# xingyizhou/CenterTrack

Hardware: AMD Instinct MI355X
Metric: frames/sec (DLA-34 + DCNv2 CenterTrack hot path: H2D of the frame + forward + decode + D2H + track association) (higher is better)
Workload: dtype f32; 1 GPU; mot17_512: mot heads, DLA-34, 512x512, 1 stream(s)/GPU, K=100, flip_test=False, seeded random-init weights; one step = 64 consecutive frames of every stream, each frame uploaded from pinned host memory inside the step (frame t+1 on a copy stream while frame t runs); global_batch=1, parallelism=streams sharded dp1, all-gather of packed detections, hip_graph=True

## Files before the change

centertrack_amd/_lib.py:

```python
import ctypes
import os

_PKG = os.path.dirname(os.path.abspath(__file__))
LIB_PATH = os.environ.get('CENTERTRACK_LIB') or os.path.join(_PKG, 'libcentertrack_hip.so')

c_float_p = ctypes.c_void_p
NUM_HEADS = 11
(HEAD_REG, HEAD_WH, HEAD_TRACKING, HEAD_LTRB, HEAD_LTRB_AMODAL, HEAD_DEP, HEAD_ROT, HEAD_DIM,
 HEAD_AMODEL_OFFSET, HEAD_NUSCENES_ATT, HEAD_VELOCITY) = range(NUM_HEADS)
HEAD_INDEX = {'reg': HEAD_REG, 'wh': HEAD_WH, 'tracking': HEAD_TRACKING, 'ltrb': HEAD_LTRB,
              'ltrb_amodal': HEAD_LTRB_AMODAL, 'dep': HEAD_DEP, 'rot': HEAD_ROT, 'dim': HEAD_DIM,
              'amodel_offset': HEAD_AMODEL_OFFSET, 'nuscenes_att': HEAD_NUSCENES_ATT,
              'velocity': HEAD_VELOCITY}
HEAD_CH = {'reg': 2, 'wh': 2, 'tracking': 2, 'ltrb': 4, 'ltrb_amodal': 4, 'dep': 1, 'rot': 8, 'dim': 3,
           'amodel_offset': 2, 'nuscenes_att': 8, 'velocity': 3}

CT_RELU = 1
CT_OUT_NCHW = 2
CT_DCN_MAIN, CT_DCN_FINISH, CT_DCN_OFFSETS = 1, 2, 4
CT_OK, CT_ERR_ARG, CT_ERR_LAUNCH, CT_ERR_WORKSPACE = 0, 1, 2, 3


class ConvDesc(ctypes.Structure):
    _fields_ = [('x', ctypes.c_void_p), ('N', ctypes.c_int), ('H', ctypes.c_int), ('W', ctypes.c_int),
# ... 142 lines not shown
                ('frame', ctypes.c_void_p), ('next_frame', ctypes.c_void_p),
                ('trans_input', ctypes.c_void_p), ('trans_inv', ctypes.c_void_p)]


CT_FRAME_DEVICE, CT_FRAME_HOST, CT_FRAME_IN_PLACE, CT_FRAME_UPLOADED = range(4)


ABI_VERSION = 103

EXPORTS = ['ct_last_error', 'ct_version', 'ct_set_tuning', 'ct_packed_weight_elems', 'ct_pack_conv_weight',
           'ct_packed_winograd_elems', 'ct_pack_winograd_weight', 'ct_conv2d',
           'ct_conv2d_workspace_bytes', 'ct_heads_fused', 'ct_dcn_v2', 'ct_dcn_v2_workspace_bytes', 'ct_dcn_v2_offsets_bytes', 'ct_dcn_v2_group', 'ct_dcn_v2_group_workspace_bytes', 'ct_dcn_v2_group_plan',
           'ct_dcn_v2_backward', 'ct_dcn_v2_backward_workspace_bytes', 'ct_packed_dcn_weight_t_elems', 'ct_pack_dcn_weight_t', 'ct_stem_forward',
           'ct_maxpool2x2', 'ct_upsample_add', 'ct_nchw_to_nhwc', 'ct_nhwc_to_nchw',
           'ct_decode_row_floats', 'ct_decode_workspace_bytes', 'ct_decode', 'ct_decode_pose_workspace_bytes',
           'ct_decode_pose', 'ct_render_pre_hm',
           'ct_tracker_create', 'ct_tracker_destroy', 'ct_tracker_reset', 'ct_tracker_num_tracks',
           'ct_tracker_id_count', 'ct_tracker_get_tracks', 'ct_tracker_step', 'ct_tracker_prehm_params', 'ct_linear_assignment', 'ct_tracker_set_mode', 'ct_tracker_init_tracks',
           'ct_tracker_step_public', 'ct_tracker_step_dets', 'ct_transform_points',
           'ct_preprocess_image', 'ct_preprocess_lut', 'ct_preprocess_device', 'ct_graph_begin', 'ct_graph_end', 'ct_graph_launch', 'ct_graph_destroy',
           'ct_memcpy_async', 'ct_memset_async', 'ct_stream_synchronize', 'ct_flip_merge', 'ct_flip_images',
           'ct_frame_loop_create', 'ct_frame_loop_destroy', 'ct_frame_loop_submit', 'ct_frame_loop_wait', 'ct_frame_loop_finish',
           'ct_frame_loop_finish_submit', 'ct_frame_loop_upload', 'ct_frame_loop_pending_slot', 'ct_frame_loop_in_flight',
           'ct_frame_loop_forget_upload', 'ct_frame_loop_prestage', 'ct_stem_forward_parts', 'ct_signal_host']

_lib = None


class CTError(RuntimeError):
    pass


def load():
    global _lib
    if _lib is not None:
        return _lib
    if not os.path.exists(LIB_PATH):
        raise CTError('%s not found: build it with `python -c "import __graft_entry__ as g; g.build()"` '
                      '(hipcc --offload-arch=gfx950); there is no CPU fallback' % LIB_PATH)
    import torch
    lib = ctypes.CDLL(LIB_PATH)
    i, p, sz = ctypes.c_int, ctypes.c_void_p, ctypes.c_size_t
    lib.ct_last_error.restype = ctypes.c_char_p
    lib.ct_version.restype = i
    if lib.ct_version() != ABI_VERSION:
        raise CTError('%s is ABI version %d, this binding was written against %d: rebuild it (python -m '
                      'centertrack_amd.build)' % (LIB_PATH, lib.ct_version(), ABI_VERSION))
# ... 5 lines not shown
    lib.ct_packed_winograd_elems.argtypes = [i, i]
    lib.ct_pack_winograd_weight.argtypes = [p, p, i, i, p]
    lib.ct_conv2d.argtypes = [ctypes.POINTER(ConvDesc), p]
    lib.ct_conv2d_workspace_bytes.restype = sz
    lib.ct_conv2d_workspace_bytes.argtypes = [ctypes.POINTER(ConvDesc)]
    lib.ct_heads_fused.argtypes = [ctypes.POINTER(HeadsDesc), p]
    lib.ct_dcn_v2.argtypes = [ctypes.POINTER(DcnDesc), p]
    lib.ct_dcn_v2_workspace_bytes.restype = sz
    lib.ct_dcn_v2_workspace_bytes.argtypes = [ctypes.POINTER(DcnDesc)]
    lib.ct_dcn_v2_offsets_bytes.restype = sz
    lib.ct_dcn_v2_offsets_bytes.argtypes = [ctypes.POINTER(DcnDesc)]
    lib.ct_dcn_v2_group.argtypes = [ctypes.POINTER(DcnDesc), i, i, p]
    lib.ct_dcn_v2_group_workspace_bytes.restype = sz
    lib.ct_dcn_v2_group_workspace_bytes.argtypes = [ctypes.POINTER(DcnDesc)]
    lib.ct_dcn_v2_group_plan.argtypes = [ctypes.POINTER(DcnDesc), ctypes.POINTER(ctypes.c_size_t), ctypes.POINTER(ctypes.c_int)]
    lib.ct_dcn_v2_backward.argtypes = [ctypes.POINTER(DcnBwdDesc), p]
    lib.ct_dcn_v2_backward_workspace_bytes.restype = sz
    lib.ct_dcn_v2_backward_workspace_bytes.argtypes = [ctypes.POINTER(DcnBwdDesc)]
    lib.ct_packed_dcn_weight_t_elems.restype = sz
    lib.ct_packed_dcn_weight_t_elems.argtypes = [i, i]
    lib.ct_pack_dcn_weight_t.argtypes = [p, p, i, i, p]
    lib.ct_stem_forward.argtypes = [p, p, p, i, i, i, p, p, p, p, p, p, i, p]
    lib.ct_stem_forward_parts.argtypes = [p, p, p, p, i, i, i, i, p, p, p, p, p, p, i, p]
    lib.ct_maxpool2x2.argtypes = [p, i, i, i, i, i, p, i, p]
    lib.ct_upsample_add.argtypes = [p, i, i, i, i, i, p, i, p, i, p, i, p]
    lib.ct_nchw_to_nhwc.argtypes = [p, i, i, i, i, p, i, p]
    lib.ct_nhwc_to_nchw.argtypes = [p, i, i, i, i, i, p, p]
    lib.ct_decode_row_floats.argtypes = [ctypes.POINTER(DecodeDesc)]
    lib.ct_decode_workspace_bytes.restype = sz
    lib.ct_decode_workspace_bytes.argtypes = [ctypes.POINTER(DecodeDesc)]
    lib.ct_decode.argtypes = [ctypes.POINTER(DecodeDesc), p]
    lib.ct_decode_pose_workspace_bytes.restype = sz
    lib.ct_decode_pose_workspace_bytes.argtypes = [ctypes.POINTER(PoseDesc)]
    lib.ct_decode_pose.argtypes = [ctypes.POINTER(PoseDesc), p]
    lib.ct_render_pre_hm.argtypes = [p, p, i, i, i, i, p, i, p]
    lib.ct_tracker_create.restype = p
    lib.ct_tracker_create.argtypes = [ctypes.c_float, i]
    lib.ct_tracker_destroy.restype = None
    lib.ct_tracker_destroy.argtypes = [p]
    lib.ct_tracker_reset.restype = None
    lib.ct_tracker_reset.argtypes = [p]
    lib.ct_tracker_num_tracks.argtypes = [p]
    lib.ct_tracker_id_count.argtypes = [p]
    lib.ct_tracker_get_tracks.argtypes = [p, p, i]
    lib.ct_tracker_step.argtypes = [p, p, i, i, ctypes.POINTER(RowLayout), ctypes.c_float, p, p, i]
    lib.ct_tracker_prehm_params.argtypes = [p, ctypes.c_float, p, i, i, p, i]
# ... 74 lines not shown
```

centertrack_amd/csrc/stem.hip:

```cpp
#include "ct_common.h"

namespace {

constexpr int ST_TW = 32;
constexpr int ST_PW = 40;
template <int TH> struct StCfg {
    static constexpr int PH = TH + 6;
    static constexpr int PS = PH * ST_PW;
    static constexpr int NPV = (3 * PH * 38 + 255) / 256;
    static constexpr int HALVES = TH / 8;
};
__host__ __device__ constexpr int st_k4(int s) { return s == 2 ? 52 : 148; }
__host__ __device__ constexpr int st_koff(int s) { return s * 148; }
constexpr int ST_KTOT = 348;
constexpr int ST_WLP = 16;

CT_DEFINE_STAMPS(stem)

struct StemArgs {
    const float *in[3];
    const float *w[3];
    const float *scale;
    const float *shift;
    const float *add;
    float *y;
    int N, H, W, ldy, ldadd, tilesX, tilesY;
};

constexpr int ST_NWV = 10;

template <int TH>
__attribute__((amdgpu_waves_per_eu(TH == 16 ? 2 : 1)))
__global__ __launch_bounds__(256) void stem_kernel(StemArgs a)
{
    using SC = StCfg<TH>;
    constexpr int ST_TH = TH, ST_PH = SC::PH, ST_PS = SC::PS, ST_NPV = SC::NPV, MT = 4, HV = SC::HALVES;
    __shared__ __attribute__((aligned(16))) float planes[7 * ST_PS];
    __shared__ __attribute__((aligned(16))) float wl[ST_KTOT * ST_WLP];
    __shared__ int tab[ST_KTOT];
    CT_STAMP_RT(0);
    CT_STAMP(1);
    CT_STAMP_HW(8);

    const int tid = threadIdx.x;
    const int lane = tid & 63, wave = __builtin_amdgcn_readfirstlane(tid >> 6);
    const int li = lane & 15, lg = lane >> 4;
    int bid = blockIdx.x;
    const int tx = bid % a.tilesX; bid /= a.tilesX;
    const int ty = bid % a.tilesY; bid /= a.tilesY;
    const int n = bid;
    const int oy0 = ty * ST_TH, ox0 = tx * ST_TW;
    const size_t HW = (size_t)a.H * a.W;

    for (int k = tid; k < ST_KTOT; k += 256) {
        const int s = (k >= 296) ? 2 : ((k >= 148) ? 1 : 0);
        const int kk = k - st_koff(s);
        const int cin = (s == 2) ? 1 : 3;
        int off = 0;
        if (kk < cin * 49) {
            const int c = kk / 49, r = kk - c * 49;
            off = (3 * s + c) * ST_PS + (r / 7) * ST_PW + (r % 7);
        }
        tab[k] = off;
    }

    float pv[ST_NPV], wv[ST_NWV];
    auto stage_load = [&](int s) {
        const int cin = (s == 2) ? 1 : 3;
        const int K = cin * 49;
        const float *src = a.in[s] + (size_t)n * cin * HW;
        const float *w = a.w[s];
        const int np = cin * ST_PH * 38, nw = st_k4(s) * 16;
#pragma unroll
        for (int i = 0; i < ST_NPV; ++i) {
            const int it = tid + 256 * i;
            const int c = it / (ST_PH * 38);
            const int r = it - c * (ST_PH * 38);
            const int py = r / 38, px = r - py * 38;
            const int iy = oy0 - 3 + py, ix = ox0 - 3 + px;
            const bool ok = it < np && iy >= 0 && iy < a.H && ix >= 0 && ix < a.W;
            const float v = src[ok ? ((size_t)c * HW + (size_t)iy * a.W + ix) : 0];
            pv[i] = ok ? v : 0.0f;
        }
#pragma unroll
        for (int i = 0; i < ST_NWV; ++i) {
            const int it = tid + 256 * i;
            const int k = it >> 4, j = it & 15;
            const bool ok = it < nw && k < K;
            const float v = w[ok ? (j * K + k) : 0];
            wv[i] = ok ? v : 0.0f;
        }
    };
    auto stage_store = [&](int s) {
        const int cin = (s == 2) ? 1 : 3;
        const int np = cin * ST_PH * 38, nw = st_k4(s) * 16;
#pragma unroll
        for (int i = 0; i < ST_NPV; ++i) {
            const int it = tid + 256 * i;
            if (it < np) {
                const int c = it / (ST_PH * 38);
                const int r = it - c * (ST_PH * 38);
                const int py = r / 38, px = r - py * 38;
                planes[(3 * s + c) * ST_PS + py * ST_PW + px] = pv[i];
            }
        }
#pragma unroll
        for (int i = 0; i < ST_NWV; ++i) {
            const int it = tid + 256 * i;
            if (it < nw) wl[st_koff(s) * 16 + it] = wv[i];
        }
    };

    int pbase[MT];
#pragma unroll
    for (int mt = 0; mt < MT; ++mt) pbase[mt] = (2 * wave + (mt >> 1)) * ST_PW + (mt & 1) * 16 + li;

    f32x4 out[HV][MT];
#pragma unroll
    for (int h = 0; h < HV; ++h)
#pragma unroll
    for (int mt = 0; mt < MT; ++mt) {
        out[h][mt] = f32x4{0.f, 0.f, 0.f, 0.f};
        if (a.add) {
            const int oy = oy0 + 8 * h + 2 * wave + (mt >> 1);
#pragma unroll
            for (int e = 0; e < 4; ++e) {
                const int ox = ox0 + (mt & 1) * 16 + lg * 4 + e;
                if (oy < a.H && ox < a.W) out[h][mt][e] = a.add[(((size_t)n * a.H + oy) * a.W + ox) * a.ldadd + li];
            }
        }
    }

    const int first = a.in[0] ? 0 : (a.in[1] ? 1 : 2);
    stage_load(first);
    CT_STAMP(2);
    stage_store(first);
    __syncthreads();
    CT_STAMP(3);
#pragma unroll
    for (int s = 0; s < 3; ++s) {
        if (s < first) continue;
        const int nxt = (s < 1 && a.in[1]) ? 1 : ((s < 2 && a.in[2]) ? 2 : 3);
        const bool have_next = a.in[s] != nullptr && nxt < 3;
        if (have_next) stage_load(nxt);
        if (a.in[s]) {
            const float sc = a.scale[s * 16 + li], sh = a.shift[s * 16 + li];
#pragma unroll
            for (int h = 0; h < HV; ++h) {
                f32x4 acc[MT];
#pragma unroll
                for (int mt = 0; mt < MT; ++mt) acc[mt] = f32x4{0.f, 0.f, 0.f, 0.f};
                const int nsteps = st_k4(s) / 4;
#pragma unroll 4
                for (int st = 0; st < nsteps; ++st) {
                    const int k = st_koff(s) + 4 * st + lg;
                    const int off = tab[k] + 8 * h * ST_PW;
                    const float b = wl[k * ST_WLP + li];
#pragma unroll
                    for (int mt = 0; mt < MT; ++mt)
                        acc[mt] = __builtin_amdgcn_mfma_f32_16x16x4f32(planes[off + pbase[mt]], b, acc[mt], 0, 0, 0);
                }
#pragma unroll
                for (int mt = 0; mt < MT; ++mt)
#pragma unroll
                    for (int e = 0; e < 4; ++e) out[h][mt][e] += fmaxf(acc[mt][e] * sc + sh, 0.0f);
            }
        }
        if (have_next) stage_store(nxt);
        if (s < 2) __syncthreads();
        if (s == 0) CT_STAMP(4);
        if (s == 1) CT_STAMP(5);
    }
    CT_STAMP(9);

#pragma unroll
    for (int h = 0; h < HV; ++h)
#pragma unroll
    for (int mt = 0; mt < MT; ++mt) {
        const int oy = oy0 + 8 * h + 2 * wave + (mt >> 1);
        if (oy >= a.H) continue;
#pragma unroll
        for (int e = 0; e < 4; ++e) {
            const int ox = ox0 + (mt & 1) * 16 + lg * 4 + e;
            if (ox < a.W) a.y[(((size_t)n * a.H + oy) * a.W + ox) * a.ldy + li] = out[h][mt][e];
        }
    }
    CT_STAMP(6);
    CT_STAMP_RT(7);
}

}

extern "C" int ct_stem_forward(const float *x, const float *pre_img, const float *pre_hm, int N, int H, int W,
                               const float *w_x, const float *w_img, const float *w_hm, const float *scale3,
                               const float *shift3, float *y, int ldy, void *stream)
{
    if (!x) CT_FAIL_ARG("ct_stem_forward: null pointer");
    return ct_stem_forward_parts(x, pre_img, pre_hm, nullptr, 0, N, H, W, w_x, w_img, w_hm, scale3, shift3, y, ldy, stream);
}

extern "C" int ct_stem_forward_parts(const float *x, const float *pre_img, const float *pre_hm, const float *add, int ldadd,
                                     int N, int H, int W, const float *w_x, const float *w_img, const float *w_hm,
                                     const float *scale3, const float *shift3, float *y, int ldy, void *stream)
{
    if (!scale3 || !shift3 || !y) CT_FAIL_ARG("ct_stem_forward: null pointer");
    if (!x && !pre_img && !pre_hm) CT_FAIL_ARG("ct_stem_forward_parts: no stem selected");
    if ((x && !w_x) || (pre_img && !w_img) || (pre_hm && !w_hm)) CT_FAIL_ARG("ct_stem_forward: input given without its weights");
    if (N <= 0 || H <= 0 || W <= 0 || ldy < 16 || (add && ldadd < 16)) CT_FAIL_ARG("ct_stem_forward: bad shape");
    StemArgs a;
    a.in[0] = x; a.in[1] = pre_img; a.in[2] = pre_hm;
    a.w[0] = w_x; a.w[1] = w_img; a.w[2] = w_hm;
    a.scale = scale3; a.shift = shift3; a.y = y; a.add = add; a.ldadd = ldadd;
    a.N = N; a.H = H; a.W = W; a.ldy = ldy;
    a.tilesX = ct_cdiv(W, ST_TW);
    const long blocks8 = (long)N * a.tilesX * ct_cdiv(H, 8);
    const int want = ct_tune_get(CT_TUNE_STEM_ROWS);
    const bool rows16 = want == 16 || (want == 0 && blocks8 > 768 && blocks8 <= 1536);
    a.tilesY = ct_cdiv(H, rows16 ? 16 : 8);
    const long blocks = (long)N * a.tilesX * a.tilesY;
    if (blocks > 0x7fffffffL) CT_FAIL_ARG("ct_stem_forward: grid too large");
    if (rows16) hipLaunchKernelGGL(stem_kernel<16>, dim3((unsigned)blocks), dim3(256), 0, (hipStream_t)stream, a);
    else hipLaunchKernelGGL(stem_kernel<8>, dim3((unsigned)blocks), dim3(256), 0, (hipStream_t)stream, a);
    CT_CHECK_LAUNCH("ct_stem_forward");
    return CT_OK;
}
```

centertrack_amd/detector.py:

```python
import ctypes
import math
import os
import time

import numpy as np
import torch

from . import _lib, fast_track, ops
NATIVE_LOOP = os.environ.get('CENTERTRACK_NATIVE_LOOP', '1') != '0'
SPLIT_STEM_MAX = int(os.environ.get('CENTERTRACK_SPLIT_STEM_MAX', '0'))
HOST_FLAG = os.environ.get('CENTERTRACK_HOST_FLAG', '1') != '0'
HOST_ROWS = os.environ.get('CENTERTRACK_HOST_ROWS', '1') != '0'
from .image import (affine_transform, draw_umich_gaussian, gaussian_radius, get_affine_transform, make_meta)
from .model import create_model, load_model
from .post_process import generic_post_process
from .tracker import Tracker

MEAN = np.array([0.40789654, 0.44719302, 0.47026115], dtype=np.float32).reshape(1, 1, 3)
STD = np.array([0.28863828, 0.27408164, 0.27809835], dtype=np.float32).reshape(1, 1, 3)
REST_FOCAL_LENGTH = {'nuscenes': 1200, 'kitti': 721.5377, 'kitti_tracking': 721.5377}
AVERAGE_FLIPS = ('hm', 'wh', 'dep', 'dim')
NEG_AVERAGE_FLIPS = ('amodel_offset',)
COCO_FLIP_IDX = [[1, 2], [3, 4], [5, 6], [7, 8], [9, 10], [11, 12], [13, 14], [15, 16]]


def trans_bbox(bbox, trans, width, height):
    bbox = np.array(bbox, dtype=np.float32).copy()
    bbox[:2] = affine_transform(bbox[:2], trans)
    bbox[2:] = affine_transform(bbox[2:], trans)
    bbox[[0, 2]] = np.clip(bbox[[0, 2]], 0, width - 1)
    bbox[[1, 3]] = np.clip(bbox[[1, 3]], 0, height - 1)
    return bbox


def render_pre_hm(tracks, meta, pre_thresh, out=None, with_hm=True):
# ... 150 lines not shown
                assert v.stride(3) == 1 and v.stride(2) == v.shape[3] and v.stride(1) == v.shape[2] * v.shape[3]
                heads_arr[i].src, heads_arr[i].dst = v.data_ptr(), m.data_ptr()
                heads_arr[i].src_batch_stride, heads_arr[i].C, heads_arr[i].mode = v.stride(0), v.shape[1], mode
            pairs = np.ascontiguousarray(getattr(opt, 'flip_idx', COCO_FLIP_IDX), np.int32).reshape(-1, 2)
            hm0 = outs['hm']
            ctx['flip_call'] = (heads_arr, len(fl), pairs, int(hm0.shape[2]), int(hm0.shape[3]))
        else:
            merged = outs
        ctx['merged'] = merged
        dec_heads = {k: v for k, v in merged.items() if k != 'hm'}
        ctx['done_flag'] = torch.zeros((16,), dtype=torch.int32).pin_memory()
        sparse = plan.get('sparse')
        if sparse is not None:
            sparse = dict(sparse, zero_tracking=bool(getattr(opt, 'zero_tracking', False)), flip=self.flip)
        F = ops.Decoder.row_floats(dec_heads, [n for n, *_ in sparse['heads']] if sparse else None)
        ctx['host_out'] = torch.zeros((merged['hm'].shape[0], opt.K, F), dtype=torch.float32).pin_memory()
        direct = HOST_FLAG and HOST_ROWS
        ctx['decoder'] = ops.Decoder(merged['hm'], dec_heads, opt.K, host_out=ctx['host_out'] if direct else None,
                                     done_flag=ctx['done_flag'] if direct else None, sparse=sparse)
        assert tuple(ctx['decoder'].out.shape) == tuple(ctx['host_out'].shape)
        ctx['host_rows'] = ctx['host_out'].numpy()
        ctx['host_hm'] = torch.zeros((NB, 1, H, W), dtype=torch.float32).pin_memory() if (with_hm and not self.native) else None
        render = self.native and with_hm
        if render:
            nblob = ctx['max_blobs'] = fast_track.max_blobs(opt.K)
            nprm = self.B * nblob * 3
            ctx['pc_host'] = torch.zeros((nprm + self.B,), dtype=torch.int32).pin_memory()
            ctx['pc_dev'] = torch.zeros((nprm + self.B,), dtype=torch.int32, device=self.device)
            ctx['prm_host'] = ctx['pc_host'][:nprm].view(self.B, nblob, 3)
            ctx['cnt_host'] = ctx['pc_host'][nprm:]
            ctx['prm_dev'] = ctx['pc_dev'][:nprm]
            ctx['cnt_dev'] = ctx['pc_dev'][nprm:]
        if self.native:
            ctx['row_layout'] = fast_track.row_layout(ctx['decoder'].layout)
        nslots = 3 if img_in is not None else 2
        ctx['nslots'] = nslots
        ctx['frames'] = [torch.zeros_like(x_in) for _ in range(nslots)]
        ctx['slot'] = 0
        ctx['graphs'] = [None] * nslots
        ctx['raw'] = False
        ctx['loop'] = None
        ctx['launched'] = None
        ctx['copy_stream'] = None
        split = img_in is not None and hm_in is not None and 0 < NB <= SPLIT_STEM_MAX
        ctx['partial'] = [ops.new_view(NB, H, W, 16, self.device) for _ in range(nslots)] if split else None

        def pre_stage(slot):
            if not split:
                return
            cur, prev = ctx['frames'][slot], ctx['frames'][(slot - 1) % nslots]
            if self.flip:
                _lib.check(_lib.load().ct_flip_images(cur.data_ptr(), cur[self.B:].data_ptr(), self.B * 3 * H, W,
                                                      _lib.stream_ptr()), 'ct_flip_images')
            self.model.run_stem_partial(cur, prev, ctx['partial'][slot])
        ctx['pre_stage'] = pre_stage

        def device_frame(slot=0, with_copies=False):
            cur = ctx['frames'][slot]
            prev = ctx['frames'][(slot - 1) % nslots] if img_in is not None else None
            if with_copies and render:
                _lib.check(_lib.load().ct_memcpy_async(ctx['pc_dev'].data_ptr(), ctx['pc_host'].data_ptr(),
                                                       ctx['pc_host'].numel() * 4, 1, _lib.stream_ptr()), 'H2D')
            lib = _lib.load()
            if render:
                _lib.check(lib.ct_render_pre_hm(ctx['prm_dev'].data_ptr(), ctx['cnt_dev'].data_ptr(),
                                                ctx['max_blobs'], self.B, H, W, hm_in.data_ptr(),
                                                1 if self.flip else 0, _lib.stream_ptr()), 'ct_render_pre_hm')
            if self.flip and not split:
                _lib.check(lib.ct_flip_images(cur.data_ptr(), cur[self.B:].data_ptr(), self.B * 3 * H, W,
                                              _lib.stream_ptr()), 'ct_flip_images')
            self.model._run_plan(plan, inputs=(cur, prev, hm_in), stem_partial=ctx['partial'][slot] if split else None)
            if self.flip:
                arr, n, pairs, h, w = ctx['flip_call']
                _lib.check(lib.ct_flip_merge(arr, n, pairs.ctypes.data, len(pairs), self.B, h, w, _lib.stream_ptr()),
                           'ct_flip_merge')
            if getattr(opt, 'zero_tracking', False) and 'tracking' in merged:
                t = merged['tracking']
                for b in range(t.shape[0]):
                    _lib.check(lib.ct_memset_async(t[b].data_ptr(), 0, t[b].numel() * 4, _lib.stream_ptr()), 'memset')
            ctx['decoder'].run()
            if with_copies and not ctx['decoder'].direct:
                _lib.check(_lib.load().ct_memcpy_async(ctx['host_out'].data_ptr(), ctx['decoder'].out.data_ptr(),
                                                       ctx['host_out'].numel() * 4, 2, _lib.stream_ptr()), 'D2H')
                if HOST_FLAG:
                    _lib.check(_lib.load().ct_signal_host(ctx['done_flag'].data_ptr(), 1, _lib.stream_ptr()), 'ct_signal_host')

        ctx['device_frame'] = device_frame
        if self.use_graph:
            try:
                torch.cuda.synchronize()
                side = torch.cuda.Stream()
                side.wait_stream(torch.cuda.current_stream())
                with torch.cuda.stream(side):
                    pre_stage(0)
                    device_frame(0)
                torch.cuda.current_stream().wait_stream(side)
                torch.cuda.synchronize()
                raw = os.environ.get('CENTERTRACK_RAW_GRAPH', '1') != '0'
                for sl in range(nslots):
                    if raw:
                        g = _HipGraph(lambda: device_frame(sl, True), collect=(sl == 0))
                    else:
                        g = torch.cuda.CUDAGraph()
                        with _lib.capture_guard(collect=False), torch.cuda.graph(g):
                            device_frame(sl)
                    ctx['graphs'][sl] = g
                ctx['raw'] = raw
# ... 266 lines not shown
                    pre_dets = metas[s].get('pre_dets', [])
                    if self.native and len(pre_dets) > 0:
                        self.fast[s].init_tracks(pre_dets)
                    if not self.native:
                        self.trackers[s].init_track(pre_dets)
            if img_in is not None:
                prev = ctx['frames'][(slot - 1) % n]
                fresh = [s for s in range(B) if not self.started[s]]
                if fresh and self.flip:
                    _lib.check(lib.ct_flip_images(fr.data_ptr(), fr[B:].data_ptr(), B * 3 * H, W, sp), 'ct_flip_images')
                if len(fresh) == B:
                    prev.copy_(fr)
                else:
                    for s in fresh:
                        prev[s].copy_(fr[s])
                        if self.flip:
                            prev[B + s].copy_(fr[B + s])
            if hm_in is not None and self.native:
                ph, ch = ctx['prm_host'].numpy(), ctx['cnt_host'].numpy()
                for s in range(B):
                    m = metas[s]
                    ch[s], _ = self.fast[s].prehm_params(opt.pre_thresh, m['trans_input'], m['inp_width'],
                                                         m['inp_height'], out=ph[s])
                if not ctx['raw']:
                    ctx['pc_dev'].copy_(ctx['pc_host'], non_blocking=True)
            elif hm_in is not None:
                hh = ctx['host_hm']
                for s in range(B):
                    render_pre_hm(self.trackers[s].tracks, metas[s], opt.pre_thresh, out=hh[s, 0].numpy(),
                                  with_hm=not getattr(opt, 'zero_pre_hm', False))
                    if self.flip:
                        hh[B + s, 0].copy_(torch.flip(hh[s, 0], [1]))
                hm_in.copy_(hh, non_blocking=True)
            for s in range(B):
                self.started[s] = True
        t1 = time.time()
        if self._rows_free is not None:
            cur.wait_event(self._rows_free)
            self._rows_free = None
        if ctx['partial'] is not None:
            if ctx['loop'] is not None:
                _lib.check(lib.ct_frame_loop_prestage(ctx['loop'], slot), 'ct_frame_loop_prestage')
            else:
                ctx['pre_stage'](slot)
        if ctx['raw']:
            ctx['graphs'][slot].replay(sp)
        elif ctx['graphs'][slot] is not None:
# ... 213 lines not shown
```

centertrack_amd/model.py:

```python
import ctypes
import os
from collections import OrderedDict

import torch

from . import _lib, autotune, ops
from .ops import View
from .weights import CHANNELS, LEVELS, dla34_param_shapes

BN_EPS = 1e-5
SMALL_SLOT_WGS = 600
FUSE_OFFSET = os.environ.get('CENTERTRACK_FUSE_OFFSET', '1') != '0'
WINOGRAD = os.environ.get('CENTERTRACK_WINOGRAD', '1') != '0'
FUSE_HEADS = os.environ.get('CENTERTRACK_FUSE_HEADS', '1') != '0'
FOLD_POOL = os.environ.get('CENTERTRACK_FOLD_POOL', '1') != '0'
FUSE_PROJ = os.environ.get('CENTERTRACK_FUSE_PROJ', '1') != '0'


def _fold_bn(sd, p):
    scale = sd[p + '.weight'].double() / torch.sqrt(sd[p + '.running_var'].double() + BN_EPS)
    shift = sd[p + '.bias'].double() - sd[p + '.running_mean'].double() * scale
    return scale.float().contiguous(), shift.float().contiguous()


# ... 391 lines not shown
                o = torch.empty((N, c, feat.H, feat.W), device=dev)
                wp, b = P[h + '.2']
                hsig = (0, c) if (fuse_sigmoid and h in ('hm', 'hm_hp')) else (0, 0)
                hdep = (0, c) if (fuse_sigmoid and h == 'dep') else (0, 0)
                d = ops.make_conv_desc(mid.slice(hc * j, hc), wp, c, 1, 1, shift=b, out_nchw=o, sig=hsig, dep=hdep,
                                       depth_scale=self.depth_scale)
                us = autotune.tune_conv(d, dev)[2] if tune else 7.0
                L.append(_Launch('heads.%s.2' % h, 'conv', d, (mid, o), us=us,
                                 ws_need=lib.ct_conv2d_workspace_bytes(ctypes.byref(d))))
                outputs[h] = o
        return OrderedDict((h, outputs[h]) for h in self.heads if h in outputs)

    def run_stem_partial(self, x, pre_img, out):
        P = self._prepare()
        lib = _lib.load()
        w = P['stem_w']
        rc = lib.ct_stem_forward_parts(x.data_ptr(), ops._p(pre_img), None, None, 0, x.shape[0], x.shape[2], x.shape[3],
                                       w[0].data_ptr(), ops._p(w[1]) if pre_img is not None else None, None,
                                       P['stem_scale'].data_ptr(), P['stem_shift'].data_ptr(), out.ptr, out.ld,
                                       _lib.stream_ptr())
        if rc != 0:
            _lib.check(rc, 'stem (x / pre_img terms)')

    def _run_plan(self, plan, inputs=None, stem_partial=None, launches=None):
        P = self._prepared
        lib = _lib.load()
        st = _lib.stream_ptr()
        for l in (plan['launches'] if launches is None else launches):
            if l.fn == 'conv':
                rc = lib.ct_conv2d(ctypes.byref(l.args), st)
            elif l.fn == 'dcn_group':
                arr, n, phases = l.args
                rc = lib.ct_dcn_v2_group(arr, n, phases, st)
            elif l.fn == 'heads':
                rc = lib.ct_heads_fused(ctypes.byref(l.args), st)
            elif l.fn == 'pool':
                x, y = l.args
                rc = lib.ct_maxpool2x2(x.ptr, x.N, x.H, x.W, x.C, x.ld, y.ptr, y.ld, st)
            elif l.fn == 'stem':
                x, img, hm, y = l.args
                if inputs is not None:
                    x, img, hm = inputs
                w = P['stem_w']
                if stem_partial is not None:
                    if hm is None:
                        raise _lib.CTError('a split stem needs the pre_hm input')
                    rc = lib.ct_stem_forward_parts(None, None, hm.data_ptr(), stem_partial.ptr, stem_partial.ld,
                                                   x.shape[0], x.shape[2], x.shape[3], None, None, w[2].data_ptr(),
                                                   P['stem_scale'].data_ptr(), P['stem_shift'].data_ptr(), y.ptr, y.ld, st)
                    if rc != 0:
                        _lib.check(rc, l.name)
                    continue
                rc = lib.ct_stem_forward(x.data_ptr(), ops._p(img), ops._p(hm), x.shape[0], x.shape[2], x.shape[3],
                                         w[0].data_ptr(), ops._p(w[1]) if img is not None else None,
                                         ops._p(w[2]) if hm is not None else None,
                                         P['stem_scale'].data_ptr(), P['stem_shift'].data_ptr(), y.ptr, y.ld, st)
            else:
                raise AssertionError(l.fn)
            if rc != 0:
                _lib.check(rc, l.name)

    def _schedule_dcn(self, layers, produced0, N, dev, knobs, tune=True):
        lib = _lib.load()
        P = self._prepared
        fuse_max_cin, cps, nkk = knobs[:3]
        split_offsets = knobs[3] if len(knobs) > 3 else 1
# ... 312 lines not shown
```

centertrack_amd/ops.py:

```python
import ctypes

import torch

from . import _lib
from ._lib import CT_OUT_NCHW, CT_RELU, ConvDesc, DcnBwdDesc, DcnDesc, DecodeDesc


class View(object):
    __slots__ = ('buf', 'c0', 'C')

    def __init__(self, buf, c0=0, C=None):
        assert buf.dim() == 4 and buf.is_contiguous() and buf.dtype == torch.float32
        self.buf = buf
        self.c0 = c0
        self.C = buf.shape[3] - c0 if C is None else C
        assert 0 <= c0 and c0 + self.C <= buf.shape[3]

    N = property(lambda s: s.buf.shape[0])
    H = property(lambda s: s.buf.shape[1])
    W = property(lambda s: s.buf.shape[2])
    ld = property(lambda s: s.buf.shape[3])
    ptr = property(lambda s: s.buf.data_ptr() + 4 * s.c0)

    def slice(self, c0, C):
# ... 192 lines not shown
        return None, None, None, None
    if (need_x or need_om) and wT is None:
        raise _lib.CTError('dcn_v2_backward: the input / offset / mask gradients need the transposed weight packing')
    gx = new_view(x.N, x.H, x.W, x.C, dev) if need_x else None
    gom = View(torch.empty((x.N, x.H, x.W, 32), dtype=torch.float32, device=dev), 0, 27) if need_om else None
    gw = torch.empty((gy.C, x.C, 3, 3), dtype=torch.float32, device=dev) if need_w or need_b else None
    gb = torch.empty(gy.C, dtype=torch.float32, device=dev) if need_b else None
    d = make_dcn_bwd_desc(x, om, gy, wT, gx, gom, gw, gb)
    need = lib.ct_dcn_v2_backward_workspace_bytes(ctypes.byref(d))
    if need:
        ws = torch.empty(need // 4, dtype=torch.float32, device=dev)
        d.workspace, d.workspace_bytes = ws.data_ptr(), need
    _lib.check(lib.ct_dcn_v2_backward(ctypes.byref(d), _lib.stream_ptr()), 'ct_dcn_v2_backward')
    return gx, gom, (gw if need_w else None), gb


def stem(x, pre_img, pre_hm, w_x, w_img, w_hm, scale3, shift3, out=None):
    N, _, H, W = x.shape
    if out is None:
        out = new_view(N, H, W, 16, x.device)
    _lib.check(_lib.load().ct_stem_forward(
        x.data_ptr(), _p(pre_img), _p(pre_hm), N, H, W, w_x.data_ptr(), _p(w_img), _p(w_hm),
        scale3.data_ptr(), shift3.data_ptr(), out.ptr, out.ld, _lib.stream_ptr()), 'ct_stem_forward')
    return out


def maxpool2x2(x, out=None):
    if out is None:
        out = new_view(x.N, x.H // 2, x.W // 2, x.C, x.buf.device)
    _lib.check(_lib.load().ct_maxpool2x2(x.ptr, x.N, x.H, x.W, x.C, x.ld, out.ptr, out.ld, _lib.stream_ptr()),
               'ct_maxpool2x2')
    return out


def upsample_weight(w):
    return w.reshape(w.shape[0], -1).t().contiguous()


def upsample_add(x, w, f, skip, out=None):
    if w.dim() == 4:
        w = upsample_weight(w)
    if out is None:
        out = new_view(x.N, x.H * f, x.W * f, x.C, x.buf.device)
    _lib.check(_lib.load().ct_upsample_add(x.ptr, x.N, x.H, x.W, x.C, x.ld, w.data_ptr(), f, skip.ptr, skip.ld,
                                           out.ptr, out.ld, _lib.stream_ptr()), 'ct_upsample_add')
    return out
# ... 135 lines not shown
```

include/centertrack_hip.h:

```cpp
#ifndef CENTERTRACK_HIP_H
#define CENTERTRACK_HIP_H

#include <stddef.h>
#include <stdint.h>

#ifdef __cplusplus
extern "C" {
#endif

#define CT_OK 0
#define CT_ERR_ARG 1
#define CT_ERR_LAUNCH 2
#define CT_ERR_WORKSPACE 3

#define CT_RELU 1
#define CT_OUT_NCHW 2

#define CT_ABI_VERSION 103

const char *ct_last_error(void);
int ct_version(void);
int ct_set_tuning(const char *key, int value);

size_t ct_packed_weight_elems(int Cout, int Cin, int ks);
// ... 65 lines not shown
typedef struct ct_dcn_bwd_desc {
    const float *x; int N, H, W, Cin, ldx;
    const float *om; int ldom;
    const float *gy; int Cout, ldgy;
    const float *wT_packed;
    float *gx; int ldgx;
    float *gom; int ldgom;
    float *gw; float *gb;
    float *workspace; size_t workspace_bytes;
    int flags;
} ct_dcn_bwd_desc;
int ct_dcn_v2_backward(const ct_dcn_bwd_desc *d, void *stream);
size_t ct_dcn_v2_backward_workspace_bytes(const ct_dcn_bwd_desc *d);
size_t ct_packed_dcn_weight_t_elems(int Cout, int Cin);
int ct_pack_dcn_weight_t(const float *w_oihw, float *packed, int Cout, int Cin, void *stream);

int ct_stem_forward(const float *x, const float *pre_img, const float *pre_hm, int N, int H, int W,
                    const float *w_x, const float *w_img, const float *w_hm,
                    const float *scale3, const float *shift3,
                    float *y, int ldy, void *stream);
int ct_stem_forward_parts(const float *x, const float *pre_img, const float *pre_hm, const float *add, int ldadd,
                          int N, int H, int W, const float *w_x, const float *w_img, const float *w_hm,
                          const float *scale3, const float *shift3, float *y, int ldy, void *stream);

int ct_maxpool2x2(const float *x, int N, int H, int W, int C, int ldx, float *y, int ldy, void *stream);
int ct_upsample_add(const float *x, int N, int H, int W, int C, int ldx, const float *w, int f,
                    const float *skip, int lds, float *y, int ldy, void *stream);
int ct_nchw_to_nhwc(const float *x, int N, int C, int H, int W, float *y, int ldy, void *stream);
int ct_nhwc_to_nchw(const float *x, int N, int C, int H, int W, int ldx, float *y, void *stream);

enum { CT_HEAD_REG = 0, CT_HEAD_WH, CT_HEAD_TRACKING, CT_HEAD_LTRB, CT_HEAD_LTRB_AMODAL,
       CT_HEAD_DEP, CT_HEAD_ROT, CT_HEAD_DIM, CT_HEAD_AMODEL_OFFSET, CT_HEAD_NUSCENES_ATT,
       CT_HEAD_VELOCITY, CT_NUM_HEADS };
typedef struct ct_sparse_heads_desc {
    const float *feat; int ldf;
    int nheads;
    int head[CT_NUM_HEADS];
    const float *w1[CT_NUM_HEADS], *b1[CT_NUM_HEADS], *w2[CT_NUM_HEADS], *b2[CT_NUM_HEADS];
    float depth_scale;
    int zero_tracking;
    int flip_B;
    int flip_mode[CT_NUM_HEADS];
} ct_sparse_heads_desc;
typedef struct ct_decode_desc {
    const float *hm; int B, C, h, w, K;
    const float *heads[CT_NUM_HEADS];
// ... 137 lines not shown
```

Baseline: 1146 frames/s.

## Fuse pre_hm gaussian rendering into the stem kernel, reading blobs from host

The stem kernel gains a blob mode: rather than loading a rendered pre_hm plane, each tile culls the blob list to those overlapping its halo, compacts them into shared memory, and renders the gaussian peaks straight into the third input plane. This removes the separate render_pre_hm kernel, the full-resolution heatmap write and read, and by default the H2D copy of blob params, since the kernel reads the pinned host buffer directly. The costs are per-tile double-precision exp work, extra barriers and shared memory in the stem, and reads over the host link from inside the kernel.

```diff
diff --git a/centertrack_amd/_lib.py b/centertrack_amd/_lib.py
--- a/centertrack_amd/_lib.py
+++ b/centertrack_amd/_lib.py
@@ -188,7 +188,8 @@
            'ct_memcpy_async', 'ct_memset_async', 'ct_stream_synchronize', 'ct_flip_merge', 'ct_flip_images',
            'ct_frame_loop_create', 'ct_frame_loop_destroy', 'ct_frame_loop_submit', 'ct_frame_loop_wait', 'ct_frame_loop_finish',
            'ct_frame_loop_finish_submit', 'ct_frame_loop_upload', 'ct_frame_loop_pending_slot', 'ct_frame_loop_in_flight',
-           'ct_frame_loop_forget_upload', 'ct_frame_loop_prestage', 'ct_stem_forward_parts', 'ct_signal_host']
+           'ct_frame_loop_forget_upload', 'ct_frame_loop_prestage', 'ct_stem_forward_parts', 'ct_signal_host',
+           'ct_stem_forward_blobs']
 
 _lib = None
 
@@ -240,6 +241,7 @@
     lib.ct_pack_dcn_weight_t.argtypes = [p, p, i, i, p]
     lib.ct_stem_forward.argtypes = [p, p, p, i, i, i, p, p, p, p, p, p, i, p]
     lib.ct_stem_forward_parts.argtypes = [p, p, p, p, i, i, i, i, p, p, p, p, p, p, i, p]
+    lib.ct_stem_forward_blobs.argtypes = [p, p, p, p, i, i, p, i, i, i, i, p, p, p, p, p, p, i, p]
     lib.ct_maxpool2x2.argtypes = [p, i, i, i, i, i, p, i, p]
     lib.ct_upsample_add.argtypes = [p, i, i, i, i, i, p, i, p, i, p, i, p]
     lib.ct_nchw_to_nhwc.argtypes = [p, i, i, i, i, p, i, p]
diff --git a/centertrack_amd/csrc/stem.hip b/centertrack_amd/csrc/stem.hip
--- a/centertrack_amd/csrc/stem.hip
+++ b/centertrack_amd/csrc/stem.hip
@@ -14,6 +14,7 @@
 __host__ __device__ constexpr int st_koff(int s) { return s * 148; }
 constexpr int ST_KTOT = 348;
 constexpr int ST_WLP = 16;
+constexpr int ST_BCAP = 256;
 
 CT_DEFINE_STAMPS(stem)
 
@@ -25,11 +26,14 @@
     const float *add;
     float *y;
     int N, H, W, ldy, ldadd, tilesX, tilesY;
+    const int *bp;
+    const int *bc;
+    int cap, nstreams;
 };
 
 constexpr int ST_NWV = 10;
 
-template <int TH>
+template <int TH, bool BL>
 __attribute__((amdgpu_waves_per_eu(TH == 16 ? 2 : 1)))
 __global__ __launch_bounds__(256) void stem_kernel(StemArgs a)
 {
@@ -38,6 +42,8 @@
     __shared__ __attribute__((aligned(16))) float planes[7 * ST_PS];
     __shared__ __attribute__((aligned(16))) float wl[ST_KTOT * ST_WLP];
     __shared__ int tab[ST_KTOT];
+    __shared__ int blob[BL ? ST_BCAP * 3 : 1];
+    __shared__ int nblob;
     CT_STAMP_RT(0);
     CT_STAMP(1);
     CT_STAMP_HW(8);
@@ -51,12 +57,18 @@
     const int n = bid;
     const int oy0 = ty * ST_TH, ox0 = tx * ST_TW;
     const size_t HW = (size_t)a.H * a.W;
-
+    const bool mirrored = BL && n >= a.nstreams;
+    const int bstream = mirrored ? n - a.nstreams : n;
+    int bn = 0, bcx = 0, bcy = 0, br = -1;
+    if constexpr (BL) bn = min(a.bc[bstream], a.cap);
+    auto has = [&](int s) { return a.in[s] != nullptr || (BL && s == 2); };
+
+    const int pad_off = (a.in[0] ? 0 : (a.in[1] ? 3 : 6)) * ST_PS;
     for (int k = tid; k < ST_KTOT; k += 256) {
         const int s = (k >= 296) ? 2 : ((k >= 148) ? 1 : 0);
         const int kk = k - st_koff(s);
         const int cin = (s == 2) ? 1 : 3;
-        int off = 0;
+        int off = pad_off;
         if (kk < cin * 49) {
             const int c = kk / 49, r = kk - c * 49;
             off = (3 * s + c) * ST_PS + (r / 7) * ST_PW + (r % 7);
@@ -71,16 +83,23 @@
         const float *src = a.in[s] + (size_t)n * cin * HW;
         const float *w = a.w[s];
         const int np = cin * ST_PH * 38, nw = st_k4(s) * 16;
-#pragma unroll
-        for (int i = 0; i < ST_NPV; ++i) {
-            const int it = tid + 256 * i;
-            const int c = it / (ST_PH * 38);
-            const int r = it - c * (ST_PH * 38);
-            const int py = r / 38, px = r - py * 38;
-            const int iy = oy0 - 3 + py, ix = ox0 - 3 + px;
-            const bool ok = it < np && iy >= 0 && iy < a.H && ix >= 0 && ix < a.W;
-            const float v = src[ok ? ((size_t)c * HW + (size_t)iy * a.W + ix) : 0];
-            pv[i] = ok ? v : 0.0f;
+        if (BL && s == 2) {
+            if (tid < bn) {
+                const int *p = a.bp + ((size_t)bstream * a.cap + tid) * 3;
+                bcx = p[0]; bcy = p[1]; br = p[2];
+            }
+        } else {
+#pragma unroll
+            for (int i = 0; i < ST_NPV; ++i) {
+                const int it = tid + 256 * i;
+                const int c = it / (ST_PH * 38);
+                const int r = it - c * (ST_PH * 38);
+                const int py = r / 38, px = r - py * 38;
+                const int iy = oy0 - 3 + py, ix = ox0 - 3 + px;
+                const bool ok = it < np && iy >= 0 && iy < a.H && ix >= 0 && ix < a.W;
+                const float v = src[ok ? ((size_t)c * HW + (size_t)iy * a.W + ix) : 0];
+                pv[i] = ok ? v : 0.0f;
+            }
         }
 #pragma unroll
         for (int i = 0; i < ST_NWV; ++i) {
@@ -91,17 +110,76 @@
             wv[i] = ok ? v : 0.0f;
         }
     };
+    auto render_store = [&]() {
+        const int ylo = oy0 - 3, yhi = oy0 - 3 + ST_PH - 1;
+        const int pxlo = ox0 - 3, pxhi = ox0 - 3 + 37;
+        const int xlo = mirrored ? a.W - 1 - pxhi : pxlo, xhi = mirrored ? a.W - 1 - pxlo : pxhi;
+        for (int c0 = 0; c0 == 0 || c0 < bn; c0 += ST_BCAP) {
+            const int c1 = min(bn, c0 + ST_BCAP);
+            if (tid == 0) nblob = 0;
+            __syncthreads();
+            {
+                const int i = c0 + tid;
+                int cx = bcx, cy = bcy, r = br;
+                if (c0 > 0) {
+                    r = -1;
+                    if (i < c1) {
+                        const int *p = a.bp + ((size_t)bstream * a.cap + i) * 3;
+                        cx = p[0]; cy = p[1]; r = p[2];
+                    }
+                }
+                const bool hit = i < c1 && r >= 0 && cx + r >= xlo && cx - r <= xhi && cy + r >= ylo && cy - r <= yhi;
+                const unsigned long long mask = __ballot(hit);
+                int base = 0;
+                if (mask) {
+                    const int leader = __ffsll((long long)mask) - 1;
+                    if (lane == leader) base = atomicAdd(&nblob, (int)__popcll(mask));
+                    base = __shfl(base, leader);
+                }
+                if (hit) {
+                    const int q = base + (int)__popcll(mask & ((1ull << lane) - 1ull));
+                    blob[3 * q] = cx; blob[3 * q + 1] = cy; blob[3 * q + 2] = r;
+                }
+            }
+            __syncthreads();
+            const int m = nblob;
+#pragma unroll 1
+            for (int it = tid; it < ST_PH * 38; it += 256) {
+                const int py = it / 38, px = it - py * 38;
+                const int iy = ylo + py, ix = pxlo + px;
+                const bool ok = iy >= 0 && iy < a.H && ix >= 0 && ix < a.W;
+                const int x = mirrored ? a.W - 1 - ix : ix, y = iy;
+                float *dst = &planes[6 * ST_PS + py * ST_PW + px];
+                float v = c0 > 0 ? *dst : 0.0f;
+                const int mi = ok ? m : 0;
+                for (int j = 0; j < mi; ++j) {
+                    const int cx = blob[3 * j], cy = blob[3 * j + 1], r = blob[3 * j + 2];
+                    const int dx = x - cx, dy = y - cy;
+                    if (dx < -r || dx > r || dy < -r || dy > r) continue;
+                    const double sigma = (double)(2 * r + 1) / 6.0;
+                    const double g = exp(-(double)(dx * dx + dy * dy) / (2.0 * sigma * sigma));
+                    v = fmaxf(v, (float)g);
+                }
+                *dst = v;
+            }
+            if (c0 + ST_BCAP < bn) __syncthreads();
+        }
+    };
     auto stage_store = [&](int s) {
         const int cin = (s == 2) ? 1 : 3;
         const int np = cin * ST_PH * 38, nw = st_k4(s) * 16;
-#pragma unroll
-        for (int i = 0; i < ST_NPV; ++i) {
-            const int it = tid + 256 * i;
-            if (it < np) {
-                const int c = it / (ST_PH * 38);
-                const int r = it - c * (ST_PH * 38);
-                const int py = r / 38, px = r - py * 38;
-                planes[(3 * s + c) * ST_PS + py * ST_PW + px] = pv[i];
+        if (BL && s == 2) {
+            render_store();
+        } else {
+#pragma unroll
+            for (int i = 0; i < ST_NPV; ++i) {
+                const int it = tid + 256 * i;
+                if (it < np) {
+                    const int c = it / (ST_PH * 38);
+                    const int r = it - c * (ST_PH * 38);
+                    const int py = r / 38, px = r - py * 38;
+                    planes[(3 * s + c) * ST_PS + py * ST_PW + px] = pv[i];
+                }
             }
         }
 #pragma unroll
@@ -140,10 +218,10 @@
 #pragma unroll
     for (int s = 0; s < 3; ++s) {
         if (s < first) continue;
-        const int nxt = (s < 1 && a.in[1]) ? 1 : ((s < 2 && a.in[2]) ? 2 : 3);
-        const bool have_next = a.in[s] != nullptr && nxt < 3;
+        const int nxt = (s < 1 && a.in[1]) ? 1 : ((s < 2 && has(2)) ? 2 : 3);
+        const bool have_next = has(s) && nxt < 3;
         if (have_next) stage_load(nxt);
-        if (a.in[s]) {
+        if (has(s)) {
             const float sc = a.scale[s * 16 + li], sh = a.shift[s * 16 + li];
 #pragma unroll
             for (int h = 0; h < HV; ++h) {
@@ -187,6 +265,28 @@
     }
     CT_STAMP(6);
     CT_STAMP_RT(7);
+}
+
+int stem_launch(StemArgs &a, const char *what, void *stream)
+{
+    a.tilesX = ct_cdiv(a.W, ST_TW);
+    const long blocks8 = (long)a.N * a.tilesX * ct_cdiv(a.H, 8);
+    const int want = ct_tune_get(CT_TUNE_STEM_ROWS);
+    const bool rows16 = want == 16 || (want == 0 && blocks8 > 768 && blocks8 <= 1536);
+    a.tilesY = ct_cdiv(a.H, rows16 ? 16 : 8);
+    const long blocks = (long)a.N * a.tilesX * a.tilesY;
+    if (blocks > 0x7fffffffL) CT_FAIL_ARG("%s: grid too large", what);
+    const dim3 grid((unsigned)blocks), wg(256);
+    hipStream_t st = (hipStream_t)stream;
+    if (a.bp) {
+        if (rows16) hipLaunchKernelGGL((stem_kernel<16, true>), grid, wg, 0, st, a);
+        else hipLaunchKernelGGL((stem_kernel<8, true>), grid, wg, 0, st, a);
+    } else {
+        if (rows16) hipLaunchKernelGGL((stem_kernel<16, false>), grid, wg, 0, st, a);
+        else hipLaunchKernelGGL((stem_kernel<8, false>), grid, wg, 0, st, a);
+    }
+    CT_CHECK_LAUNCH(what);
+    return CT_OK;
 }
 
 }
@@ -212,15 +312,24 @@
     a.w[0] = w_x; a.w[1] = w_img; a.w[2] = w_hm;
     a.scale = scale3; a.shift = shift3; a.y = y; a.add = add; a.ldadd = ldadd;
     a.N = N; a.H = H; a.W = W; a.ldy = ldy;
-    a.tilesX = ct_cdiv(W, ST_TW);
-    const long blocks8 = (long)N * a.tilesX * ct_cdiv(H, 8);
-    const int want = ct_tune_get(CT_TUNE_STEM_ROWS);
-    const bool rows16 = want == 16 || (want == 0 && blocks8 > 768 && blocks8 <= 1536);
-    a.tilesY = ct_cdiv(H, rows16 ? 16 : 8);
-    const long blocks = (long)N * a.tilesX * a.tilesY;
-    if (blocks > 0x7fffffffL) CT_FAIL_ARG("ct_stem_forward: grid too large");
-    if (rows16) hipLaunchKernelGGL(stem_kernel<16>, dim3((unsigned)blocks), dim3(256), 0, (hipStream_t)stream, a);
-    else hipLaunchKernelGGL(stem_kernel<8>, dim3((unsigned)blocks), dim3(256), 0, (hipStream_t)stream, a);
-    CT_CHECK_LAUNCH("ct_stem_forward");
-    return CT_OK;
-}
+    a.bp = nullptr; a.bc = nullptr; a.cap = 0; a.nstreams = N;
+    return stem_launch(a, "ct_stem_forward", stream);
+}
+
+extern "C" int ct_stem_forward_blobs(const float *x, const float *pre_img, const int *params, const int *counts, int cap,
+                                     int mirrored, const float *add, int ldadd, int N, int H, int W, const float *w_x,
+                                     const float *w_img, const float *w_hm, const float *scale3, const float *shift3,
+                                     float *y, int ldy, void *stream)
+{
+    if (!params || !counts || !w_hm || !scale3 || !shift3 || !y) CT_FAIL_ARG("ct_stem_forward_blobs: null pointer");
+    if ((x && !w_x) || (pre_img && !w_img)) CT_FAIL_ARG("ct_stem_forward_blobs: input given without its weights");
+    if (N <= 0 || H <= 0 || W <= 0 || cap <= 0 || ldy < 16 || (add && ldadd < 16)) CT_FAIL_ARG("ct_stem_forward_blobs: bad shape");
+    if (mirrored && (N & 1)) CT_FAIL_ARG("ct_stem_forward_blobs: a mirrored batch holds an even number of images");
+    StemArgs a;
+    a.in[0] = x; a.in[1] = pre_img; a.in[2] = nullptr;
+    a.w[0] = w_x; a.w[1] = w_img; a.w[2] = w_hm;
+    a.scale = scale3; a.shift = shift3; a.y = y; a.add = add; a.ldadd = ldadd;
+    a.N = N; a.H = H; a.W = W; a.ldy = ldy;
+    a.bp = params; a.bc = counts; a.cap = cap; a.nstreams = mirrored ? N / 2 : N;
+    return stem_launch(a, "ct_stem_forward_blobs", stream);
+}
diff --git a/centertrack_amd/detector.py b/centertrack_amd/detector.py
--- a/centertrack_amd/detector.py
+++ b/centertrack_amd/detector.py
@@ -11,6 +11,8 @@
 SPLIT_STEM_MAX = int(os.environ.get('CENTERTRACK_SPLIT_STEM_MAX', '0'))
 HOST_FLAG = os.environ.get('CENTERTRACK_HOST_FLAG', '1') != '0'
 HOST_ROWS = os.environ.get('CENTERTRACK_HOST_ROWS', '1') != '0'
+STEM_RENDER = os.environ.get('CENTERTRACK_STEM_RENDER', '1') != '0'
+STEM_BLOBS_HOST = os.environ.get('CENTERTRACK_STEM_BLOBS', 'host') != 'device'
 from .image import (affine_transform, draw_umich_gaussian, gaussian_radius, get_affine_transform, make_meta)
 from .model import create_model, load_model
 from .post_process import generic_post_process
@@ -207,6 +209,9 @@
         ctx['host_rows'] = ctx['host_out'].numpy()
         ctx['host_hm'] = torch.zeros((NB, 1, H, W), dtype=torch.float32).pin_memory() if (with_hm and not self.native) else None
         render = self.native and with_hm
+        fused = render and STEM_RENDER
+        blobs_host = fused and STEM_BLOBS_HOST
+        ctx['blobs_host'] = blobs_host
         if render:
             nblob = ctx['max_blobs'] = fast_track.max_blobs(opt.K)
             nprm = self.B * nblob * 3
@@ -243,31 +248,46 @@
         def device_frame(slot=0, with_copies=False):
             cur = ctx['frames'][slot]
             prev = ctx['frames'][(slot - 1) % nslots] if img_in is not None else None
-            if with_copies and render:
+            rec = ctx['frame_launches'] = []
+            if with_copies and render and not blobs_host:
+                rec.append('H2D blobs')
                 _lib.check(_lib.load().ct_memcpy_async(ctx['pc_dev'].data_ptr(), ctx['pc_host'].data_ptr(),
                                                        ctx['pc_host'].numel() * 4, 1, _lib.stream_ptr()), 'H2D')
             lib = _lib.load()
-            if render:
+            if render and not fused:
+                rec.append('ct_render_pre_hm')
                 _lib.check(lib.ct_render_pre_hm(ctx['prm_dev'].data_ptr(), ctx['cnt_dev'].data_ptr(),
                                                 ctx['max_blobs'], self.B, H, W, hm_in.data_ptr(),
                                                 1 if self.flip else 0, _lib.stream_ptr()), 'ct_render_pre_hm')
             if self.flip and not split:
+                rec.append('ct_flip_images')
                 _lib.check(lib.ct_flip_images(cur.data_ptr(), cur[self.B:].data_ptr(), self.B * 3 * H, W,
                                               _lib.stream_ptr()), 'ct_flip_images')
-            self.model._run_plan(plan, inputs=(cur, prev, hm_in), stem_partial=ctx['partial'][slot] if split else None)
+            blobs = None
+            if fused:
+                src = ('prm_host', 'cnt_host') if blobs_host else ('prm_dev', 'cnt_dev')
+                blobs = (ctx[src[0]].data_ptr(), ctx[src[1]].data_ptr(), ctx['max_blobs'], self.flip)
+            self.model._run_plan(plan, inputs=(cur, prev, hm_in), stem_partial=ctx['partial'][slot] if split else None,
+                                 blobs=blobs)
+            rec.extend(l.name for l in plan['launches'])
             if self.flip:
+                rec.append('ct_flip_merge')
                 arr, n, pairs, h, w = ctx['flip_call']
                 _lib.check(lib.ct_flip_merge(arr, n, pairs.ctypes.data, len(pairs), self.B, h, w, _lib.stream_ptr()),
                            'ct_flip_merge')
             if getattr(opt, 'zero_tracking', False) and 'tracking' in merged:
                 t = merged['tracking']
                 for b in range(t.shape[0]):
+                    rec.append('memset tracking')
                     _lib.check(lib.ct_memset_async(t[b].data_ptr(), 0, t[b].numel() * 4, _lib.stream_ptr()), 'memset')
+            rec.append('decode')
             ctx['decoder'].run()
             if with_copies and not ctx['decoder'].direct:
+                rec.append('D2H rows')
                 _lib.check(_lib.load().ct_memcpy_async(ctx['host_out'].data_ptr(), ctx['decoder'].out.data_ptr(),
                                                        ctx['host_out'].numel() * 4, 2, _lib.stream_ptr()), 'D2H')
                 if HOST_FLAG:
+                    rec.append('ct_signal_host')
                     _lib.check(_lib.load().ct_signal_host(ctx['done_flag'].data_ptr(), 1, _lib.stream_ptr()), 'ct_signal_host')
 
         ctx['device_frame'] = device_frame
@@ -580,7 +600,7 @@
                     m = metas[s]
                     ch[s], _ = self.fast[s].prehm_params(opt.pre_thresh, m['trans_input'], m['inp_width'],
                                                          m['inp_height'], out=ph[s])
-                if not ctx['raw']:
+                if not ctx['raw'] and not ctx['blobs_host']:
                     ctx['pc_dev'].copy_(ctx['pc_host'], non_blocking=True)
             elif hm_in is not None:
                 hh = ctx['host_hm']
diff --git a/centertrack_amd/model.py b/centertrack_amd/model.py
--- a/centertrack_amd/model.py
+++ b/centertrack_amd/model.py
@@ -437,7 +437,7 @@
         if rc != 0:
             _lib.check(rc, 'stem (x / pre_img terms)')
 
-    def _run_plan(self, plan, inputs=None, stem_partial=None, launches=None):
+    def _run_plan(self, plan, inputs=None, stem_partial=None, launches=None, blobs=None):
         P = self._prepared
         lib = _lib.load()
         st = _lib.stream_ptr()
@@ -457,6 +457,20 @@
                 if inputs is not None:
                     x, img, hm = inputs
                 w = P['stem_w']
+                if blobs is not None:
+                    if hm is None:
+                        raise _lib.CTError('a blob list was given to a model without the pre_hm stem')
+                    bp, bc, cap, mirrored = blobs
+                    part = stem_partial is not None
+                    rc = lib.ct_stem_forward_blobs(None if part else x.data_ptr(), None if part else ops._p(img), bp, bc,
+                                                   cap, 1 if mirrored else 0, stem_partial.ptr if part else None,
+                                                   stem_partial.ld if part else 0, x.shape[0], x.shape[2], x.shape[3],
+                                                   None if part else w[0].data_ptr(),
+                                                   ops._p(w[1]) if (img is not None and not part) else None, w[2].data_ptr(),
+                                                   P['stem_scale'].data_ptr(), P['stem_shift'].data_ptr(), y.ptr, y.ld, st)
+                    if rc != 0:
+                        _lib.check(rc, l.name)
+                    continue
                 if stem_partial is not None:
                     if hm is None:
                         raise _lib.CTError('a split stem needs the pre_hm input')
diff --git a/centertrack_amd/ops.py b/centertrack_amd/ops.py
--- a/centertrack_amd/ops.py
+++ b/centertrack_amd/ops.py
@@ -238,6 +238,21 @@
     _lib.check(_lib.load().ct_stem_forward(
         x.data_ptr(), _p(pre_img), _p(pre_hm), N, H, W, w_x.data_ptr(), _p(w_img), _p(w_hm),
         scale3.data_ptr(), shift3.data_ptr(), out.ptr, out.ld, _lib.stream_ptr()), 'ct_stem_forward')
+    return out
+
+
+def stem_blobs(x, pre_img, params, counts, cap, mirrored, w_x, w_img, w_hm, scale3, shift3, out=None, add=None):
+    if torch.is_tensor(x):
+        (N, _, H, W), dev, xp = x.shape, x.device, x.data_ptr()
+    else:
+        (N, H, W), dev, xp = x, add.buf.device, None
+    if out is None:
+        out = new_view(N, H, W, 16, dev)
+    _lib.check(_lib.load().ct_stem_forward_blobs(
+        xp, _p(pre_img), params.data_ptr(), counts.data_ptr(), cap, 1 if mirrored else 0,
+        add.ptr if add is not None else None, add.ld if add is not None else 0, N, H, W,
+        _p(w_x) if xp else None, _p(w_img) if pre_img is not None else None, w_hm.data_ptr(),
+        scale3.data_ptr(), shift3.data_ptr(), out.ptr, out.ld, _lib.stream_ptr()), 'ct_stem_forward_blobs')
     return out
 
 
diff --git a/include/centertrack_hip.h b/include/centertrack_hip.h
--- a/include/centertrack_hip.h
+++ b/include/centertrack_hip.h
@@ -111,6 +111,10 @@
 int ct_stem_forward_parts(const float *x, const float *pre_img, const float *pre_hm, const float *add, int ldadd,
                           int N, int H, int W, const float *w_x, const float *w_img, const float *w_hm,
                           const float *scale3, const float *shift3, float *y, int ldy, void *stream);
+int ct_stem_forward_blobs(const float *x, const float *pre_img, const int *params, const int *counts, int cap,
+                          int mirrored, const float *add, int ldadd, int N, int H, int W, const float *w_x,
+                          const float *w_img, const float *w_hm, const float *scale3, const float *shift3,
+                          float *y, int ldy, void *stream);
 
 int ct_maxpool2x2(const float *x, int N, int H, int W, int C, int ldx, float *y, int ldy, void *stream);
 int ct_upsample_add(const float *x, int N, int H, int W, int C, int ldx, const float *w, int f,
```

Result: no change. 1140 frames/s (-0.5%).
